# zeal-up/ORB_SLAM_Tracking

Measured on AMD Instinct MI355X. Metric: frames/sec (extract+match, 1000 feat, 640x480), higher is better.
Workload: dtype u8

## Files before the change

### orb_slam_tracking_amd/csrc/orbx_kernels.hip

```cpp
#include <hip/hip_runtime.h>

#include <algorithm>
#include <cstdint>
#include <cstdio>
#include <cstdlib>
#include <type_traits>

#include "../../include/orbx.h"
#include "orbx_launch.h"
#include "orbx_knobs.h"

namespace orbx {

__global__ __launch_bounds__(256) void k_resize(const uint8_t* __restrict__ src, long long srcFrameStride, int sw, int sh,
                                                int sstride, uint8_t* __restrict__ dst, long long dstFrameStride, int dw,
                                                int dh, int dstride, const ResizeTab* __restrict__ xtab,
                                                const ResizeTab* __restrict__ ytab) {
  const int f = blockIdx.z;
  const int dx0 = (blockIdx.x * 64 + threadIdx.x) * 4;
  const int dy = blockIdx.y * 4 + threadIdx.y;
  if (dx0 >= dw || dy >= dh) return;
  const ResizeTab ty = ytab[dy];
  const int sy0 = min(max(ty.ofs, 0), sh - 1), sy1 = min(max(ty.ofs + 1, 0), sh - 1);
  const int b0 = ty.coef & 0xffff, b1 = ty.coef >> 16;
  const uint8_t* S0 = src + (long long)f * srcFrameStride + (long long)sy0 * sstride;
  const uint8_t* S1 = src + (long long)f * srcFrameStride + (long long)sy1 * sstride;
  uint32_t packed = 0;
#pragma unroll
  for (int i = 0; i < 4; i++) {
    const ResizeTab tx = xtab[dx0 + i];
    const int sx = tx.ofs, sx1 = min(sx + 1, sw - 1);
    const int a0 = tx.coef & 0xffff, a1 = tx.coef >> 16;
    const int t0 = S0[sx] * a0 + S0[sx1] * a1;
    const int t1 = S1[sx] * a0 + S1[sx1] * a1;
    int v = (((b0 * (t0 >> 4)) >> 16) + ((b1 * (t1 >> 4)) >> 16) + 2) >> 2;
    v = min(max(v, 0), 255);
    packed |= (uint32_t)v << (8 * i);
  }
  *reinterpret_cast<uint32_t*>(dst + (long long)f * dstFrameStride + (long long)dy * dstride + dx0) = packed;
}

#define RESIZE_DW_ROWS 4
struct __attribute__((aligned(4))) PyrU3 { uint32_t a, b, c; };
__global__ __launch_bounds__(256) void k_resize_dw(const uint8_t* __restrict__ src, long long srcFrameStride, int sw, int sh,
                                                   int sstride, uint8_t* __restrict__ dst, long long dstFrameStride, int dw,
                                                   int dh, int dstride, const ResizeTab* __restrict__ xtab,
                                                   const ResizeTab* __restrict__ ytab, int wideFrames) {
  const int f = blockIdx.z;
  const int dx0 = (blockIdx.x * 64 + threadIdx.x) * 4;
  const int dyBase = blockIdx.y * (4 * RESIZE_DW_ROWS) + threadIdx.y;
  if (dx0 >= dw || dyBase >= dh) return;
  const uint4 tA = reinterpret_cast<const uint4*>(xtab + dx0)[0];
  const uint4 tB = reinterpret_cast<const uint4*>(xtab + dx0)[1];
  const int sxs[4] = {(int)tA.x, (int)tA.z, (int)tB.x, (int)tB.z};
  const uint32_t cfs[4] = {tA.y, tA.w, tB.y, tB.w};
  const int base = sxs[0] & ~3;
  const int lim = (sw - 1) & ~3;
  const int o0 = base, o1 = min(base + 4, lim), o2 = min(base + 8, lim);
  const uint8_t* S = src + (long long)f * srcFrameStride;
  uint32_t r0a[RESIZE_DW_ROWS], r0b[RESIZE_DW_ROWS], r0c[RESIZE_DW_ROWS], r1a[RESIZE_DW_ROWS], r1b[RESIZE_DW_ROWS], r1c[RESIZE_DW_ROWS];
  int b0[RESIZE_DW_ROWS], b1[RESIZE_DW_ROWS];
#pragma unroll
  for (int k = 0; k < RESIZE_DW_ROWS; k++) {
    const int dy = min(dyBase + 4 * k, dh - 1);
    const ResizeTab ty = ytab[dy];
    const int sy0 = min(max(ty.ofs, 0), sh - 1), sy1 = min(max(ty.ofs + 1, 0), sh - 1);
    b0[k] = ty.coef & 0xffff; b1[k] = ty.coef >> 16;
    const uint8_t* S0 = S + (long long)sy0 * sstride;
    const uint8_t* S1 = S + (long long)sy1 * sstride;
    if (f < wideFrames || sy1 < sh - 1) {
      const PyrU3 u0 = *reinterpret_cast<const PyrU3*>(S0 + o0), u1 = *reinterpret_cast<const PyrU3*>(S1 + o0);
      r0a[k] = u0.a; r0b[k] = u0.b; r0c[k] = u0.c;
      r1a[k] = u1.a; r1b[k] = u1.b; r1c[k] = u1.c;
    } else {
      r0a[k] = *reinterpret_cast<const uint32_t*>(S0 + o0); r0b[k] = *reinterpret_cast<const uint32_t*>(S0 + o1);
      r0c[k] = *reinterpret_cast<const uint32_t*>(S0 + o2);
      r1a[k] = *reinterpret_cast<const uint32_t*>(S1 + o0); r1b[k] = *reinterpret_cast<const uint32_t*>(S1 + o1);
      r1c[k] = *reinterpret_cast<const uint32_t*>(S1 + o2);
    }
  }
#pragma unroll
  for (int k = 0; k < RESIZE_DW_ROWS; k++) {
    const int dy = dyBase + 4 * k;
    uint32_t packed = 0;
#pragma unroll
    for (int i = 0; i < 4; i++) {
      const int kk = sxs[i] - base;
      const int sh8 = kk & 3;
      const uint32_t lo0 = kk < 4 ? r0a[k] : (kk < 8 ? r0b[k] : r0c[k]), hi0 = kk < 4 ? r0b[k] : r0c[k];
      const uint32_t lo1 = kk < 4 ? r1a[k] : (kk < 8 ? r1b[k] : r1c[k]), hi1 = kk < 4 ? r1b[k] : r1c[k];
      const uint32_t w0 = __builtin_amdgcn_alignbyte(hi0, lo0, sh8), w1 = __builtin_amdgcn_alignbyte(hi1, lo1, sh8);
      const int a0 = cfs[i] & 0xffff, a1 = cfs[i] >> 16;
      const int t0 = (int)(w0 & 255) * a0 + (int)((w0 >> 8) & 255) * a1;
      const int t1 = (int)(w1 & 255) * a0 + (int)((w1 >> 8) & 255) * a1;
      int v = (((b0[k] * (t0 >> 4)) >> 16) + ((b1[k] * (t1 >> 4)) >> 16) + 2) >> 2;
      v = min(max(v, 0), 255);
      packed |= (uint32_t)v << (8 * i);
    }
    if (dy < dh) *reinterpret_cast<uint32_t*>(dst + (long long)f * dstFrameStride + (long long)dy * dstride + dx0) = packed;
  }
}

__global__ __launch_bounds__(256) void k_pyramid_tiles(const uint8_t* __restrict__ img0, long long img0FrameStride,
                                                       uint8_t* __restrict__ pyr, const Geom g, const PyrTileRect* __restrict__ rects,
                                                       const PyrTileTap* __restrict__ taps, int buf0Bytes, int bufBytes) {
  extern __shared__ __attribute__((aligned(16))) uint8_t tileLds[];
  PyrTileTap* T = reinterpret_cast<PyrTileTap*>(tileLds);
  uint8_t* buf0 = tileLds + ORBX_PYR_TILE_TAPS * sizeof(PyrTileTap);
  uint8_t* bufA = buf0 + buf0Bytes;
  uint8_t* bufB = bufA + bufBytes;
  const int f = blockIdx.y + g.frame0, t = blockIdx.x;
  const PyrTileRect* __restrict__ R = rects + (size_t)t * g.nlevels;
  {
    int nT = 0;
    for (int l = 1; l < g.nlevels; l++) nT += (R[l].nx1 - R[l].nx0) + (R[l].ny1 - R[l].ny0);
    const uint2* __restrict__ src = reinterpret_cast<const uint2*>(taps + (size_t)t * ORBX_PYR_TILE_TAPS);
    uint2* dst = reinterpret_cast<uint2*>(T);
    uint2 tv[ORBX_PYR_TILE_TAPS / 256];
#pragma unroll
    for (int q = 0; q < ORBX_PYR_TILE_TAPS / 256; q++) tv[q] = (int)threadIdx.x + q * 256 < nT ? src[threadIdx.x + q * 256] : make_uint2(0, 0);
    const PyrTileRect R0 = R[0];
    const int w0 = R0.nx1 - R0.nx0, n0 = w0 * (R0.ny1 - R0.ny0);
    const uint32_t inv0 = ((1u << 20) + (uint32_t)w0 - 1) / (uint32_t)max(w0, 1);
    const uint8_t* G0 = img0 + (long long)f * img0FrameStride + (long long)R0.ny0 * g.L[0].stride + R0.nx0;
    for (int base = 0; base < n0; base += 8 * 256) {
      uint8_t pv[8];
#pragma unroll
      for (int q = 0; q < 8; q++) {
        const int idx = min(base + q * 256 + (int)threadIdx.x, n0 - 1);
        const int y = (int)(((uint32_t)idx * inv0) >> 20), x = idx - y * w0;
        pv[q] = G0[(long long)y * g.L[0].stride + x];
      }
#pragma unroll
      for (int q = 0; q < 8; q++)
        if (base + q * 256 + (int)threadIdx.x < n0) buf0[base + q * 256 + threadIdx.x] = pv[q];
    }
#pragma unroll
    for (int q = 0; q < ORBX_PYR_TILE_TAPS / 256; q++)
      if ((int)threadIdx.x + q * 256 < nT) dst[threadIdx.x + q * 256] = tv[q];
  }
  __syncthreads();
  const uint8_t* srcL = buf0;
  int ppitch = R[0].nx1 - R[0].nx0;
  uint8_t* dstL = bufA;
  int tapOff = 0;
  for (int l = 1; l < g.nlevels; l++) {
    const LevelGeom& D = g.L[l];
    const PyrTileRect Rl = R[l];
    const int nw = Rl.nx1 - Rl.nx0, nh = Rl.ny1 - Rl.ny0, npx = nw * nh;
    const uint32_t inv = ((1u << 20) + (uint32_t)nw - 1) / (uint32_t)max(nw, 1);
    const PyrTileTap* TX = T + tapOff;
    const PyrTileTap* TY = TX + nw;
    uint8_t* out = pyr + D.imgOff + (long long)f * D.frameStride;
    for (int base = 0; base < npx; base += 4 * 256) {
      int pi[4], pj[4];
      PyrTileTap ex[4], ey[4];
#pragma unroll
      for (int q = 0; q < 4; q++) {
        const int idx = min(base + q * 256 + (int)threadIdx.x, npx - 1);
        pj[q] = (int)(((uint32_t)idx * inv) >> 20);
        pi[q] = idx - pj[q] * nw;
        ex[q] = TX[pi[q]];
        ey[q] = TY[pj[q]];
      }
      int p00[4], p01[4], p10[4], p11[4];
#pragma unroll
      for (int q = 0; q < 4; q++) {
        const uint8_t* S0 = srcL + (int)(ey[q].pos & 0xffff) * ppitch + (int)(ex[q].pos & 0xffff);
        const uint8_t* S1 = S0 + (int)(ey[q].pos >> 16) * ppitch;
        const int d = (int)(ex[q].pos >> 16);
        p00[q] = S0[0]; p01[q] = S0[d]; p10[q] = S1[0]; p11[q] = S1[d];
      }
#pragma unroll
      for (int q = 0; q < 4; q++) {
        const int a0 = ex[q].coef & 0xffff, a1 = ex[q].coef >> 16, b0 = ey[q].coef & 0xffff, b1 = ey[q].coef >> 16;
        const int t0 = p00[q] * a0 + p01[q] * a1;
        const int t1 = p10[q] * a0 + p11[q] * a1;
        int v = (((b0 * (t0 >> 4)) >> 16) + ((b1 * (t1 >> 4)) >> 16) + 2) >> 2;
        v = min(max(v, 0), 255);
        if (base + q * 256 + (int)threadIdx.x < npx) {
          dstL[pj[q] * nw + pi[q]] = (uint8_t)v;
          const int x = Rl.nx0 + pi[q], y = Rl.ny0 + pj[q];
          if (y >= Rl.oy0 && y < Rl.oy1 && x >= Rl.ox0 && x < Rl.ox1) out[(long long)y * D.stride + x] = (uint8_t)v;
        }
      }
    }
    __syncthreads();
    tapOff += nw + nh;
    ppitch = nw;
    srcL = dstL;
    dstL = (dstL == bufA) ? bufB : bufA;
  }
}

typedef unsigned short ushort2v __attribute__((ext_vector_type(2)));
__device__ __forceinline__ uint32_t dot2u16(uint32_t a, uint32_t b, uint32_t c) {
  return __builtin_amdgcn_udot2(__builtin_bit_cast(ushort2v, a), __builtin_bit_cast(ushort2v, b), c, false);
}

__device__ __forceinline__ uint32_t mulHiU24(uint32_t a, uint32_t b) {
  return (uint32_t)(((unsigned long long)(a & 0xffffffu) * (unsigned long long)(b & 0xffffffu)) >> 32);
}
#define PYR_T 512
#define PYR_R 2
template <int DUAL2, int GMAX>
__global__ __launch_bounds__(PYR_T) void k_pyramid_bands(const uint8_t* __restrict__ img0, long long img0FrameStride,
                                                       uint8_t* __restrict__ pyr, const Geom g,
                                                       const uint4* __restrict__ ptab, const PyrBands pb) {
  extern __shared__ uint4 yrows[];
  const int f = blockIdx.y + g.frame0, strip = (int)blockIdx.x / pb.nBands, band = (int)blockIdx.x - strip * pb.nBands, tid = threadIdx.x;
  const int nl = g.nlevels;
  struct Cols {
    uint32_t o[GMAX], sel[GMAX][6], cf[GMAX][4];
    int G, rpp, rsub, col, gOff;
    bool lanes, haveG[GMAX];
  };
  auto loadCols = [&](int l, Cols& c) {
    c.gOff = pb.g0[strip][l];
    const int ng = max(pb.g1[strip][l] - c.gOff, 1);
    const int ngt2 = (ng + 1) >> 1;
    const int use1 = ng <= PYR_T ? ng * (PYR_T / ng) : 0, use2 = ngt2 * (PYR_T / ngt2);
    c.G = GMAX == 2 && use2 > use1 ? 2 : 1;
    const int ngt = c.G == 2 ? ngt2 : ng;
    c.rpp = max(PYR_T / ngt, 1);
    c.rsub = tid / ngt;
    c.col = tid - c.rsub * ngt;
    c.lanes = c.rsub < c.rpp;
    const uint4* xg = ptab + pb.xoff[l];
#pragma unroll
    for (int j = 0; j < GMAX; j++) {
      const int gx = c.col * c.G + j;
      c.haveG[j] = c.lanes && j < c.G && gx < pb.g1[strip][l] - c.gOff;
      const uint4* e = xg + (unsigned)(c.haveG[j] ? c.gOff + gx : 0) * 4u;
      const uint4 X0 = e[0], X1 = e[1], X2 = e[2];
      const uint32_t X3 = e[3].x;
      c.o[j] = X0.x;
      c.sel[j][0] = X0.w; c.sel[j][1] = X1.x; c.sel[j][2] = X1.y; c.sel[j][3] = X1.z; c.sel[j][4] = X1.w; c.sel[j][5] = X2.x;
      c.cf[j][0] = X2.y; c.cf[j][1] = X2.z; c.cf[j][2] = X2.w; c.cf[j][3] = X3;
    }
  };
  Cols C;
  loadCols(1, C);
  {
    const int r0 = pb.r0[band][1], n = pb.r1[band][1] - r0;
    if (tid < n) yrows[pb.maxRows + tid] = (ptab + pb.yoff[1])[r0 + tid];
  }
  __syncthreads();
  for (int l = 1; l < nl; l++) {
    const LevelGeom& S = g.L[l - 1];
    const LevelGeom& D = g.L[l];
    const uint8_t* src = l == 1 ? img0 + (long long)f * img0FrameStride : pyr + S.imgOff + (long long)f * S.frameStride;
    uint8_t* dst = pyr + D.imgOff + (long long)f * D.frameStride;
    const uint4* yr = yrows + (l & 1) * pb.maxRows;
    const int r0 = pb.r0[band][l], r1 = pb.r1[band][l];
    const int dstride = D.stride;
    uint4 nextY = make_uint4(0, 0, 0, 0);
    int nextN = 0;
    if (l + 1 < nl) {
      const int q0 = pb.r0[band][l + 1];
      nextN = pb.r1[band][l + 1] - q0;
      if (tid < nextN) nextY = (ptab + pb.yoff[l + 1])[q0 + tid];
    }
    const int G = C.G, rpp = C.rpp;
    static_assert(PYR_R == 2, "the row loop pairs adjacent rows");
    auto rows = [&](auto safeTag) {
    constexpr bool SAFE = decltype(safeTag)::value;
    auto load3 = [&](const uint32_t rowOff, const int j) -> PyrU3 {
      PyrU3 v;
      if (SAFE) {
        const uint32_t lim = (uint32_t)(S.w - 1) & ~3u, o0 = C.o[j], o1 = min(o0 + 4u, lim), o2 = min(o0 + 8u, lim);
        v.a = *reinterpret_cast<const uint32_t*>(src + (rowOff + o0));
        v.b = *reinterpret_cast<const uint32_t*>(src + (rowOff + o1));
        v.c = *reinterpret_cast<const uint32_t*>(src + (rowOff + o2));
      } else {
        v = *reinterpret_cast<const PyrU3*>(src + (rowOff + C.o[j]));
      }
      return v;
    };
    auto hrow = [&](const PyrU3 a, const int j, uint32_t (&t)[4]) {
      uint32_t p[4];
      p[0] = __builtin_amdgcn_perm(a.b, a.a, C.sel[j][0]);
      p[1] = __builtin_amdgcn_perm(a.b, a.a, C.sel[j][1]);
      p[2] = __builtin_amdgcn_perm(a.b, a.a, C.sel[j][2]);
      if (DUAL2) p[2] |= __builtin_amdgcn_perm(a.c, a.b, C.sel[j][3]);
      p[3] = __builtin_amdgcn_perm(a.b, a.a, C.sel[j][4]) | __builtin_amdgcn_perm(a.c, a.b, C.sel[j][5]);
#pragma unroll
      for (int i = 0; i < 4; i++) t[i] = dot2u16(p[i], C.cf[j][i], 0u) & ~0xffu;
    };
    for (int dy0 = r0 + 2 * C.rsub; dy0 < r1; dy0 += 2 * rpp) {
      const bool live0 = C.lanes && dy0 < r1, live1 = C.lanes && dy0 + 1 < r1;
      const uint4 ty0 = yr[live0 ? dy0 - r0 : 0], ty1 = yr[live1 ? dy0 + 1 - r0 : 0];
      const bool shared = ty1.x == ty0.y;
      const bool fourth = __ballot(live1 && !shared) != 0ull;
      PyrU3 ra0[GMAX], rb0[GMAX], ra1[GMAX], rb1[GMAX];
#pragma unroll
      for (int j = 0; j < GMAX; j++)
        if (j < G) {
          ra0[j] = load3(ty0.x, j);
          rb0[j] = load3(ty0.y, j);
          rb1[j] = load3(ty1.y, j);
          if (fourth) ra1[j] = load3(ty1.x, j);
        }
#pragma unroll
      for (int j = 0; j < GMAX; j++) {
        if (j >= G) continue;
        uint32_t ta0[4], tb0[4], ta1[4], tb1[4];
        hrow(ra0[j], j, ta0);
        hrow(rb0[j], j, tb0);
        hrow(rb1[j], j, tb1);
        if (fourth) {
          hrow(ra1[j], j, ta1);
#pragma unroll
          for (int i = 0; i < 4; i++) ta1[i] = shared ? tb0[i] : ta1[i];
        } else {
#pragma unroll
          for (int i = 0; i < 4; i++) ta1[i] = tb0[i];
        }
        uint32_t u[4], v[4];
#pragma unroll
        for (int i = 0; i < 4; i++) {
          u[i] = mulHiU24(ty0.z, ta0[i]) + mulHiU24(ty0.w, tb0[i]);
          v[i] = mulHiU24(ty1.z, ta1[i]) + mulHiU24(ty1.w, tb1[i]);
        }
        const uint32_t s01 = ((u[0] | (u[1] << 16)) + 0x00020002u) >> 2, s23 = ((u[2] | (u[3] << 16)) + 0x00020002u) >> 2;
        const uint32_t q01 = ((v[0] | (v[1] << 16)) + 0x00020002u) >> 2, q23 = ((v[2] | (v[3] << 16)) + 0x00020002u) >> 2;
        const unsigned col = (unsigned)((C.gOff + C.col * G + j) * 4);
        if (live0 && C.haveG[j]) *reinterpret_cast<uint32_t*>(dst + ((unsigned)(dy0 * dstride) + col)) = __builtin_amdgcn_perm(s23, s01, 0x06040200u);
        if (live1 && C.haveG[j]) *reinterpret_cast<uint32_t*>(dst + ((unsigned)((dy0 + 1) * dstride) + col)) = __builtin_amdgcn_perm(q23, q01, 0x06040200u);
      }
    }
    };
    if (l == 1 && f >= pb.safeFrom) rows(std::true_type{});
    else rows(std::false_type{});
    if (tid < nextN) yrows[((l + 1) & 1) * pb.maxRows + tid] = nextY;
    if (l + 1 < nl) loadCols(l + 1, C);
    __syncthreads();
  }
}

#define TILE_STRIDE 84
static_assert(84 * 3121 > (1 << 18) && 83 * 3121 < (1 << 18), "reciprocal of TILE_STRIDE");
#define SMAP_STRIDE 72
#define FAST_T 256
struct FastLds {
  int32_t tileBytes, smapBytes, listBytes, outCap;
};

struct Inv20Table {
  uint32_t v[80];
};
constexpr Inv20Table makeInv20() {
  Inv20Table t{};
  for (int n = 1; n < 80; n++) t.v[n] = ((1u << 20) + (uint32_t)n - 1u) / (uint32_t)n;
  return t;
}
__constant__ Inv20Table c_inv20 = makeInv20();

__device__ __forceinline__ bool arc9(uint32_t m) {
  m |= m << 16;
  uint32_t r = m & (m >> 1);
  r &= r >> 2;
  r &= r >> 4;
  r &= m >> 8;
  return (r & 0xFFFFu) != 0;
}

#define FAST_PK_BIAS 0x6500u
typedef _Float16 half2v __attribute__((ext_vector_type(2)));
__device__ __forceinline__ uint32_t fastPkMad(const uint32_t a, const uint32_t mul, const uint32_t add) {
  uint32_t r;
  asm("v_pk_mad_i16 %0, %1, %2, %3 op_sel_hi:[0,1,1]" : "=v"(r) : "v"(a), "s"(mul), "v"(add));
  return r;
}
__device__ __forceinline__ uint32_t fastStrengthBiased(const uint32_t v, const uint32_t (&p)[16]) {
  const uint32_t K = fastPkMad(v, 0xFFFF0001u, FAST_PK_BIAS * 0x00010001u);
  half2v e[16], mn3[16];
#pragma unroll
  for (int k = 0; k < 16; k++) e[k] = __builtin_bit_cast(half2v, fastPkMad(p[k], 0x0001FFFFu, K));
#pragma unroll
  for (int k = 0; k < 16; k++)
    mn3[k] = __builtin_elementwise_minimum(__builtin_elementwise_minimum(e[k], e[(k + 1) & 15]), e[(k + 2) & 15]);
  half2v R = {};
#pragma unroll
  for (int k = 0; k < 16; k += 2) {
    const half2v a0 = __builtin_elementwise_minimum(__builtin_elementwise_minimum(mn3[k], mn3[(k + 3) & 15]), mn3[(k + 6) & 15]);
    const half2v a1 = __builtin_elementwise_minimum(__builtin_elementwise_minimum(mn3[k + 1], mn3[(k + 4) & 15]), mn3[(k + 7) & 15]);
    R = k == 0 ? __builtin_elementwise_maximum(a0, a1) : __builtin_elementwise_maximum(__builtin_elementwise_maximum(R, a0), a1);
  }
  const uint32_t r = __builtin_bit_cast(uint32_t, R);
  return max(r & 0xffffu, r >> 16);
}

__global__ __launch_bounds__(FAST_T) void k_fast(const uint8_t* __restrict__ img0, long long img0FrameStride, int img0Aligned,
                                              const uint8_t* __restrict__ pyr, const Geom g,
                                              uint32_t* __restrict__ cand, int* __restrict__ cellCount,
                                              const FastLds fl) {
  extern __shared__ __attribute__((aligned(16))) uint8_t fastLds[];
  uint8_t* const tile = fastLds;
  uint8_t* const smap = fastLds + fl.tileBytes;
  uint16_t* const list = reinterpret_cast<uint16_t*>(fastLds + fl.tileBytes + fl.smapBytes);
  uint32_t* const outl = reinterpret_cast<uint32_t*>(fastLds + fl.tileBytes + fl.smapBytes + fl.listBytes);
  __shared__ int nList, nOut;

  const int t = threadIdx.x;
  const int f = blockIdx.y + g.frame0;
  int level = 0;
  const int cid = blockIdx.x;
  while (level + 1 < g.nlevels && cid >= g.L[level + 1].cellBase) level++;
  const LevelGeom& L = g.L[level];
  const int local = cid - L.cellBase;
  const int ci = (int)(((uint32_t)local * L.colsInv24) >> 24), cj = local - ci * L.nCols;
  const int iniY = ORBX_MIN_BORDER + ci * L.hCell;
  const int iniX = ORBX_MIN_BORDER + cj * L.wCell;
  int* const myCount = cellCount + (long long)f * g.nCellsTotal + cid;
  if (iniY >= L.maxBY - 3 || iniX >= L.maxBX - 6) {
    if (t == 0) *myCount = 0;
    return;
  }
  const int maxY = min(iniY + L.hCell + 6, L.maxBY), maxX = min(iniX + L.wCell + 6, L.maxBX);
  const int cw = maxX - iniX, ch = maxY - iniY;
  if (cw < 7 || ch < 7) {
    if (t == 0) *myCount = 0;
    return;
  }
  const int iw = cw - 6, ih = ch - 6;

  const uint8_t* base;
  int stride;
  bool aligned = true;
  if (level == 0) {
    base = img0 + (long long)f * img0FrameStride;
    stride = L.stride;
    aligned = img0Aligned != 0;
  } else {
    base = pyr + L.imgOff + (long long)f * L.frameStride;
    stride = L.stride;
  }
  const int ax0 = aligned ? (iniX & ~3) : iniX;
  const int xoff = iniX - ax0;
  if (aligned) {
    const int nw = (maxX - ax0 + 3) >> 2;
    const uint32_t invNw = c_inv20.v[nw];
    uint32_t* tile32 = reinterpret_cast<uint32_t*>(tile);
    const int r0 = (int)(((uint32_t)t * invNw) >> 20), c0 = t - r0 * nw;
    const int dr = (int)(((uint32_t)FAST_T * invNw) >> 20), dc = FAST_T - dr * nw;
    uint32_t goff = (uint32_t)((iniY + r0) * stride + ax0 + 4 * c0);
    const uint32_t dGoff = (uint32_t)(dr * stride + 4 * dc), wrapG = (uint32_t)(stride - 4 * nw);
    int lidx = r0 * (TILE_STRIDE / 4) + c0, c = c0;
    const int dLidx = dr * (TILE_STRIDE / 4) + dc, wrapL = TILE_STRIDE / 4 - nw;
#pragma unroll 1
    for (int idx = t; idx < nw * ch; idx += FAST_T) {
      tile32[lidx] = *reinterpret_cast<const uint32_t*>(base + goff);
      c += dc; goff += dGoff; lidx += dLidx;
      if (c >= nw) { c -= nw; goff += wrapG; lidx += wrapL; }
    }
  } else {
    const uint32_t invCw = c_inv20.v[cw];
    for (int idx = t; idx < cw * ch; idx += FAST_T) {
      const int r = (int)(((uint32_t)idx * invCw) >> 20), c = idx - r * cw;
      tile[r * TILE_STRIDE + c] = base[(long long)(iniY + r) * stride + iniX + c];
    }
  }
  {
    uint4* smap128 = reinterpret_cast<uint4*>(smap);
    for (int idx = t; idx < fl.smapBytes / 16; idx += FAST_T) smap128[idx] = make_uint4(0u, 0u, 0u, 0u);
  }
  if (t == 0) { nList = 0; nOut = 0; }
  __syncthreads();

  constexpr int RS = TILE_STRIDE;
  constexpr int ro[16] = {3 * RS,      3 * RS + 1,  2 * RS + 2,  RS + 3,  3,       -RS + 3,     -2 * RS + 2, -3 * RS + 1,
                          -3 * RS,     -3 * RS - 1, -2 * RS - 2, -RS - 3, -3,      RS - 3,      2 * RS - 2,  3 * RS - 1};
  const int py0 = (int)(((uint32_t)t * c_inv20.v[iw]) >> 20), px0 = t - py0 * iw;
  const int dpy = (int)(((uint32_t)FAST_T * c_inv20.v[iw]) >> 20), dpx = FAST_T - dpy * iw;
  const int npix = iw * ih;
  const int off0 = (py0 + 3) * TILE_STRIDE + xoff + px0 + 3, dOff = dpy * TILE_STRIDE + dpx;
  for (int pass = 0; pass < 2; pass++) {
    const int th = pass == 0 ? g.iniTh : g.minTh;
    {
      int px = px0, off = off0;
      for (int idx = t; idx < npix; idx += FAST_T) {
        const uint8_t* p = &tile[off];
        const int v = p[0], hi = v + th, lo = v - th;
        const int q0 = p[ro[0]], q4 = p[ro[4]], q8 = p[ro[8]], q12 = p[ro[12]];
        const bool b0 = q0 > hi, b4 = q4 > hi, b8 = q8 > hi, b12 = q12 > hi;
        const bool d0 = q0 < lo, d4 = q4 < lo, d8 = q8 < lo, d12 = q12 < lo;
        const bool cand0 = ((b0 | b8) & (b4 | b12)) | ((d0 | d8) & (d4 | d12));
        if (cand0) list[atomicAdd(&nList, 1)] = (uint16_t)off;
        px += dpx;
        off += dOff;
        if (px >= iw) { px -= iw; off += TILE_STRIDE - iw; }
      }
    }
    __syncthreads();
    const int nl = nList;
    for (int e = t; e < nl; e += FAST_T) {
      const int off = list[e];
      const uint8_t* p = &tile[off];
      uint32_t q[16];
#pragma unroll
      for (int k = 0; k < 16; k++) q[k] = p[ro[k]];
      const int s = (int)fastStrengthBiased(p[0], q) - (int)FAST_PK_BIAS;
      if (s > th) {
        const int row = (off * 3121) >> 18;
        smap[(row - 2) * SMAP_STRIDE + (off - row * TILE_STRIDE - xoff - 2)] = (uint8_t)s;
      } else {
        list[e] = 0xFFFF;
      }
    }
    __syncthreads();
    for (int e = t; e < nl; e += FAST_T) {
      const int off = list[e];
      if (off == 0xFFFF) continue;
      const int row = (off * 3121) >> 18;
      const int py = row - 3, px = off - row * TILE_STRIDE - xoff - 3;
      const uint8_t* q = &smap[(py + 1) * SMAP_STRIDE + px + 1];
      const int s = q[0];
      const int n0 = q[-SMAP_STRIDE - 1], n1 = q[-SMAP_STRIDE], n2 = q[-SMAP_STRIDE + 1], n3 = q[-1], n4 = q[1],
                n5 = q[SMAP_STRIDE - 1], n6 = q[SMAP_STRIDE], n7 = q[SMAP_STRIDE + 1];
      const int nmax = max(max(max(n0, n1), max(n2, n3)), max(max(n4, n5), max(n6, n7)));
      const bool keep = s > 1 && s > nmax;
      if (keep) {
        const int slot = atomicAdd(&nOut, 1);
        if (slot < fl.outCap) outl[slot] = packCand(px + 3 + cj * L.wCell, py + 3 + ci * L.hCell, s - 1);
      }
    }
    __syncthreads();
    if (nOut > 0 || pass == 1 || g.minTh >= g.iniTh) break;
    if (t == 0) nList = 0;
    __syncthreads();
  }
  const int no = min(nOut, fl.outCap);
  if (t == 0) *myCount = no;
  if (no > 0) {
    uint32_t* dstc = cand + L.candOff + (long long)f * L.candCap + (long long)local * L.segCap;
    for (int e = t; e < no; e += FAST_T) dstc[e] = outl[e];
  }
}

#define FW_RING 192
#define FW_CORN 256
#define FW_CPW 1
#define FW_XK 16

__device__ __forceinline__ int fwMbcnt(unsigned long long m) {
  return (int)__builtin_amdgcn_mbcnt_hi((uint32_t)(m >> 32), __builtin_amdgcn_mbcnt_lo((uint32_t)m, 0u));
}

typedef __attribute__((address_space(3))) uint8_t fw_lds_u8;
typedef __attribute__((address_space(3))) uint16_t fw_lds_u16;
typedef __attribute__((address_space(3))) uint32_t fw_lds_u32;
__device__ __forceinline__ const fw_lds_u8* fwLds8(const uint32_t a) { return reinterpret_cast<const fw_lds_u8*>((size_t)a); }
__device__ __forceinline__ const fw_lds_u16* fwLds16(const uint32_t a) { return reinterpret_cast<const fw_lds_u16*>((size_t)a); }
__device__ __forceinline__ const fw_lds_u32* fwLds32(const uint32_t a) { return reinterpret_cast<const fw_lds_u32*>((size_t)a); }
__device__ __forceinline__ void fwStoreB16(const uint32_t addr, const uint32_t val, const unsigned long long m) {
  unsigned long long saved;
  asm volatile("s_mov_b64 %0, exec\n\ts_mov_b64 exec, %1\n\tds_write_b16 %2, %3\n\ts_mov_b64 exec, %0"
               : "=&s"(saved)
               : "s"(m), "v"(addr), "v"(val)
               : "memory");
}
__device__ __forceinline__ void fwStoreB8(const uint32_t addr, const uint32_t val, const unsigned long long m) {
  unsigned long long saved;
  asm volatile("s_mov_b64 %0, exec\n\ts_mov_b64 exec, %1\n\tds_write_b8 %2, %3\n\ts_mov_b64 exec, %0"
               : "=&s"(saved)
               : "s"(m), "v"(addr), "v"(val)
               : "memory");
}
__device__ __forceinline__ unsigned long long fwGtLo(const uint32_t x, const uint32_t thLo) {
  unsigned long long m;
  asm("v_cmp_lt_i16_e64 %0, %1, %2" : "=s"(m) : "s"(thLo), "v"(x));
  return m;
}
__device__ __forceinline__ unsigned long long fwGtHi(const uint32_t x, const uint32_t thHi) {
  unsigned long long m;
  asm("v_cmp_lt_i32_e64 %0, %1, %2" : "=s"(m) : "s"(thHi), "v"(x));
  return m;
}

template <int TS>
__device__ __forceinline__ uint32_t fwStrength(const uint32_t e) {
  constexpr int C = 3 * TS + 3;
  constexpr int ro[16] = {C + 3 * TS,  C + 3 * TS + 1, C + 2 * TS + 2, C + TS + 3, C + 3,  C - TS + 3, C - 2 * TS + 2, C - 3 * TS + 1,
                          C - 3 * TS,  C - 3 * TS - 1, C - 2 * TS - 2, C - TS - 3, C - 3,  C + TS - 3, C + 2 * TS - 2, C + 3 * TS - 1};
  const fw_lds_u8* const p = fwLds8(e);
  uint32_t q[16];
#pragma unroll
  for (int k = 0; k < 16; k++) q[k] = p[ro[k]];
  return fastStrengthBiased(p[C], q);
}

typedef short short2v __attribute__((ext_vector_type(2)));

template <int TS>
__global__ __launch_bounds__(64) void k_fast_wave(const uint8_t* __restrict__ img0, long long img0FrameStride,
                                                  const uint8_t* __restrict__ pyr, const Geom g,
                                                  const FastCell* __restrict__ cells, uint32_t* __restrict__ cand,
                                                  int* __restrict__ cellCount, const int tileBytes, const int smapBytes) {
  extern __shared__ __attribute__((aligned(16))) uint8_t fwLds[];
  const int lane = threadIdx.x;
  uint8_t* const tile = fwLds + 16;
  uint8_t* const smap = tile + tileBytes;
  const uint32_t ldsBase = (uint32_t)(size_t)(fw_lds_u8*)fwLds;
  const uint32_t tileAddr = ldsBase + 16u, smapAddr = tileAddr + (uint32_t)tileBytes;
  const uint32_t ringAddr = smapAddr + (uint32_t)smapBytes, cornAddr = ringAddr + 2u * FW_RING;
  const uint32_t ringLane = ringAddr + 2u * (uint32_t)lane;
  const int nGroups = (g.nCellsTotal + FW_CPW - 1) / FW_CPW;
  const int xq = (int)((blockIdx.x + blockIdx.y) & 7u), xi = (int)(blockIdx.x >> 3);
  const int grp = ((xi / FW_XK) * 8 + xq) * FW_XK + (xi % FW_XK);
  if (grp >= nGroups) return;
  const int f = blockIdx.y + g.frame0;
  const int cid0 = (nGroups - 1 - grp) * FW_CPW, cid1 = min(cid0 + FW_CPW, g.nCellsTotal);
  for (int cid = cid0; cid < cid1; cid++) {
  const FastCell c = cells[cid];
  int* const myCount = cellCount + (long long)f * g.nCellsTotal + cid;
  const int ch = (int)(c.nw_ch >> 16);
  if (ch == 0) {
    if (lane == 0) *myCount = 0;
    continue;
  }
  const int level = (int)(c.xoff_level >> 16);
  const LevelGeom& L = g.L[level];
  const uint8_t* const base =
      (level == 0 ? img0 + (long long)f * img0FrameStride : pyr + L.imgOff + (long long)f * L.frameStride) + c.imgOff;
  {
    typedef uint32_t u32x4_a4 __attribute__((ext_vector_type(4), aligned(4)));
    constexpr int NQ = TS / 16;
    const int stride = (int)c.stride;
    if (lane < ch) {
      const uint8_t* p = base + (unsigned)(lane * stride);
      u32x4_a4 q[NQ];
#pragma unroll
// ... 2255 lines not shown
```

Before: 498,900.

## Assign contiguous row runs per subgroup and carry filtered row across pyramid iterations

```diff
diff --git a/orb_slam_tracking_amd/csrc/orbx_kernels.hip b/orb_slam_tracking_amd/csrc/orbx_kernels.hip
--- a/orb_slam_tracking_amd/csrc/orbx_kernels.hip
+++ b/orb_slam_tracking_amd/csrc/orbx_kernels.hip
@@ -263,6 +263,7 @@
     }
     const int G = C.G, rpp = C.rpp;
     static_assert(PYR_R == 2, "the row loop pairs adjacent rows");
+    constexpr bool PYR_CARRY = GMAX == 1;
     auto rows = [&](auto safeTag) {
     constexpr bool SAFE = decltype(safeTag)::value;
     auto load3 = [&](const uint32_t rowOff, const int j) -> PyrU3 {
@@ -287,34 +288,47 @@
 #pragma unroll
       for (int i = 0; i < 4; i++) t[i] = dot2u16(p[i], C.cf[j][i], 0u) & ~0xffu;
     };
-    for (int dy0 = r0 + 2 * C.rsub; dy0 < r1; dy0 += 2 * rpp) {
-      const bool live0 = C.lanes && dy0 < r1, live1 = C.lanes && dy0 + 1 < r1;
-      const uint4 ty0 = yr[live0 ? dy0 - r0 : 0], ty1 = yr[live1 ? dy0 + 1 - r0 : 0];
-      const bool shared = ty1.x == ty0.y;
-      const bool fourth = __ballot(live1 && !shared) != 0ull;
+    const int Lr = ((r1 - r0 + rpp - 1) / rpp + 1) & ~1;
+    const int run0 = r0 + C.rsub * Lr, run1 = C.lanes ? min(r1, run0 + Lr) : run0;
+    uint32_t car[GMAX][4] = {}, carOff = ~0u;
+    const unsigned col0 = (unsigned)((C.gOff + C.col * G) * 4);
+    uint8_t* out = dst + ((unsigned)(run0 * dstride) + col0);
+    const uint4* ty = yr + (run0 - r0);
+    for (int dy0 = run0; dy0 < run1; dy0 += 2, out += 2 * dstride, ty += 2) {
+      const bool live1 = dy0 + 1 < run1;
+      const uint4 ty0 = ty[0], ty1 = ty[live1 ? 1 : 0];
+      const bool upper0 = !PYR_CARRY || __ballot(ty0.x != carOff) != 0ull;
+      const bool upper1 = __ballot(live1 && ty1.x != ty0.y) != 0ull;
       PyrU3 ra0[GMAX], rb0[GMAX], ra1[GMAX], rb1[GMAX];
 #pragma unroll
       for (int j = 0; j < GMAX; j++)
         if (j < G) {
-          ra0[j] = load3(ty0.x, j);
+          if (upper0) ra0[j] = load3(ty0.x, j);
           rb0[j] = load3(ty0.y, j);
+          if (upper1) ra1[j] = load3(ty1.x, j);
           rb1[j] = load3(ty1.y, j);
-          if (fourth) ra1[j] = load3(ty1.x, j);
         }
 #pragma unroll
       for (int j = 0; j < GMAX; j++) {
         if (j >= G) continue;
         uint32_t ta0[4], tb0[4], ta1[4], tb1[4];
-        hrow(ra0[j], j, ta0);
         hrow(rb0[j], j, tb0);
         hrow(rb1[j], j, tb1);
-        if (fourth) {
+        if (upper0) {
+          hrow(ra0[j], j, ta0);
+        } else {
+#pragma unroll
+          for (int i = 0; i < 4; i++) ta0[i] = car[j][i];
+        }
+        if (upper1) {
           hrow(ra1[j], j, ta1);
-#pragma unroll
-          for (int i = 0; i < 4; i++) ta1[i] = shared ? tb0[i] : ta1[i];
         } else {
 #pragma unroll
           for (int i = 0; i < 4; i++) ta1[i] = tb0[i];
+        }
+        if (PYR_CARRY) {
+#pragma unroll
+          for (int i = 0; i < 4; i++) car[j][i] = tb1[i];
         }
         uint32_t u[4], v[4];
 #pragma unroll
@@ -324,10 +338,10 @@
         }
         const uint32_t s01 = ((u[0] | (u[1] << 16)) + 0x00020002u) >> 2, s23 = ((u[2] | (u[3] << 16)) + 0x00020002u) >> 2;
         const uint32_t q01 = ((v[0] | (v[1] << 16)) + 0x00020002u) >> 2, q23 = ((v[2] | (v[3] << 16)) + 0x00020002u) >> 2;
-        const unsigned col = (unsigned)((C.gOff + C.col * G + j) * 4);
-        if (live0 && C.haveG[j]) *reinterpret_cast<uint32_t*>(dst + ((unsigned)(dy0 * dstride) + col)) = __builtin_amdgcn_perm(s23, s01, 0x06040200u);
-        if (live1 && C.haveG[j]) *reinterpret_cast<uint32_t*>(dst + ((unsigned)((dy0 + 1) * dstride) + col)) = __builtin_amdgcn_perm(q23, q01, 0x06040200u);
-      }
+        if (C.haveG[j]) *reinterpret_cast<uint32_t*>(out + 4 * j) = __builtin_amdgcn_perm(s23, s01, 0x06040200u);
+        if (live1 && C.haveG[j]) *reinterpret_cast<uint32_t*>(out + (dstride + 4 * j)) = __builtin_amdgcn_perm(q23, q01, 0x06040200u);
+      }
+      carOff = ty1.y;
     }
     };
     if (l == 1 && f >= pb.safeFrom) rows(std::true_type{});
```

After: 511,800 (median of 6 runs). +2.6%, better.
